# nianticlabs/simplerecon

Hardware: AMD Instinct MI355X
Metric: depth frames/sec (640x480, 7 src views, 64 planes) (higher is better)
Workload: dtype f32

## Files before the change

### include/simplerecon_hip.h

```cpp
#ifndef SIMPLERECON_HIP_H_
#define SIMPLERECON_HIP_H_

#include <stddef.h>
#include <stdint.h>

#ifdef __cplusplus
extern "C" {
#endif

#define SR_OK 0
#define SR_ERR_INVALID_ARGUMENT 1
#define SR_ERR_UNSUPPORTED 2
#define SR_ERR_WORKSPACE_TOO_SMALL 3
#define SR_ERR_HIP_BASE 1000

enum {
  SR_OPT_MLP_SPLIT = 0, SR_OPT_WINO_SPLIT, SR_OPT_WINO_XCD, SR_OPT_WINO_STAGGER, SR_OPT_WINO_WG_PER_CU, SR_OPT_WINO_NT,
  SR_OPT_WINO_KSPLIT, SR_OPT_CONV_WINO, SR_OPT_CONV_TILE, SR_OPT_CONV_KSPLIT, SR_OPT_MLP_VEC_STORE, SR_OPT_MLP_XCD,
  SR_OPT_MLP_BWD_VALU, SR_OPT_T16_XCD, SR_OPT_POOL_BW, SR_OPT_POOL_XCD, SR_OPT_PW_NT, SR_OPT_PW_KS, SR_OPT_PT_CFG, SR_OPT_PT_KS,
  SR_OPT_DOT_LDS, SR_OPT_DOT_QUAD, SR_OPT_DOT_LDS_G, SR_OPT_DOT_LDS_CULL, SR_OPT_DOT_LDS_CAP, SR_OPT_UPSAMPLE_QUAD,
  SR_OPT_POOL_STREAM,
  SR_OPT_COUNT
};
int sr_option_count(void);
const char* sr_option_name(int id);
int sr_option_id(const char* name);
int sr_option_get(int id, int* value);
int sr_option_set(int id, int value, int* previous );
int sr_option_default(int id, int* value);

int sr_abi_version(void);

const char* sr_target_arch(void);


size_t sr_volume_workspace_bytes(int B, int K, int C, int h, int w);

int sr_volume_prepare(const float* src, const float* K_src, const float* T_src_cur,
                      const float* T_cur_src, int B, int K, int C, int h, int w, void* workspace,
                      size_t workspace_bytes, void* stream);

int sr_dot_volume_sweep(const float* cur, const float* invK_cur, const float* planes, int64_t ps_b,
                        int64_t ps_d, int64_t ps_y, int64_t ps_x, int B, int K, int C, int h, int w,
                        int D, float* out_cv, int64_t cv_sb, int64_t cv_sd, int64_t cv_sp,
                        float* out_lowest, uint8_t* out_mask, void* workspace,
                        size_t workspace_bytes, void* stream);

int sr_conv3x3_wino_io_nhwc_fwd(const void* in, int64_t in_batch_stride, int in_pix_stride, const float* packed_u,
                                const float* bias, const void* residual, int64_t res_batch_stride, int res_pix_stride,
                                void* out, int64_t out_batch_stride, int out_pix_stride, int B, int H, int W, int Cin,
                                int Cout, float leaky_slope, int io_dtype, void* stream);
int sr_pw_conv_io_nhwc_fwd(const void* in, int64_t in_batch_stride, int in_pix_stride, const float* packed_w,
                           const float* bias, const void* residual, int64_t res_batch_stride, int res_pix_stride, void* out,
                           int64_t out_batch_stride, int out_pix_stride, int B, int HW, int Cin, int Cout, float act_code,
                           int io_dtype, void* stream);

size_t sr_pw_conv_tiled_workspace_bytes(int M, int Cin, int Cout);
int sr_pw_conv_tiled_plan(int M, int Cin, int Cout, int can_split, int* cfg, int* ks);
int sr_pw_conv_tiled_nhwc_fwd(const float* in, int in_pix_stride, const float* packed_w, const float* bias,
                              const float* gate, const float* residual, int res_pix_stride, float* out,
                              int out_pix_stride, int M, int HW, int Cin, int Cout, float act_code, void* workspace,
                              size_t workspace_bytes, void* stream);
int sr_pw_conv_supported(int Cin, int Cout);
int sr_pw_conv_plan(int B, int HW, int Cin, int Cout, int* nt, int* ks);
int sr_pw_conv_nhwc_fwd(const float* in, int64_t in_batch_stride, int in_pix_stride, const float* packed_w,
                        const float* bias, const float* gate, const float* residual, int64_t res_batch_stride,
                        int res_pix_stride, float* out, int64_t out_batch_stride, int out_pix_stride, int B, int HW,
                        int Cin, int Cout, float act_code, void* stream);

int sr_backproject_fwd(const float* depth, const float* invK, float* out_points, int B, int h, int w, void* stream);
int sr_project3d_fwd(const float* points, const float* K, const float* T, float* out, int B, int N, float eps,
                     void* stream);
int sr_backproject_bwd(const float* grad_points, const float* invK, float* grad_depth, int B, int h, int w, void* stream);
int sr_project3d_bwd(const float* grad_out, const float* points, const float* K, const float* T, float* grad_points, int B,
                     int N, float eps, void* stream);
int sr_pose_distance_fwd(const float* T, float* out, int n, void* stream);
int sr_camera_rays_fwd(const float* points, const float* T, float* out, int B, int N, int in_camera_frame, void* stream);

int sr_selftest_rcp(const float* x, float* out_fast, float* out_div, int n, void* stream);

int sr_dot_volume_fwd(const float* cur, const float* src, const float* K_src,
                      const float* T_src_cur, const float* invK_cur, const float* planes,
                      int64_t ps_b, int64_t ps_d, int64_t ps_y, int64_t ps_x, int B, int K, int C,
                      int h, int w, int D, float* out_cv, int64_t cv_sb, int64_t cv_sd,
                      int64_t cv_sp, float* out_lowest, uint8_t* out_mask, void* workspace,
                      size_t workspace_bytes, void* stream);

int sr_warp_features_fwd(const float* src, const float* K_src, const float* T_src_cur,
                         const float* invK_cur, const float* planes, int64_t ps_b, int64_t ps_d,
                         int64_t ps_y, int64_t ps_x, int B, int K, int C, int h, int w, int Dp,
                         float* out_world, float* out_depths, float* out_warped, float* out_mask,
                         float* out_pix, void* workspace, size_t workspace_bytes, void* stream);

size_t sr_mlp_volume_workspace_bytes(int B, int K, int C, int h, int w, int hidden);

int sr_mlp_pack_weights(const float* W1, const float* b1, const float* W2, const float* b2,
                        const float* W3, const float* b3, int hidden, int B, int K, int C, int h, int w,
                        void* workspace, size_t workspace_bytes, void* stream);

int sr_mlp_volume_sweep(const float* cur, const float* invK_cur, const float* planes, int64_t ps_b,
                        int64_t ps_d, int64_t ps_y, int64_t ps_x, float leaky_slope, int B, int K,
                        int C, int h, int w, int D, float* out_cv, int64_t cv_sb, int64_t cv_sd,
                        int64_t cv_sp, float* out_lowest, uint8_t* out_mask, void* workspace,
                        size_t workspace_bytes, void* stream);

int sr_mlp_volume_fwd(const float* cur, const float* src, const float* K_src, const float* T_src_cur,
                      const float* T_cur_src, const float* invK_cur, const float* planes, int64_t ps_b,
                      int64_t ps_d, int64_t ps_y, int64_t ps_x, const float* W1, const float* b1,
                      const float* W2, const float* b2, const float* W3, const float* b3, int hidden,
                      float leaky_slope, int B, int K, int C, int h, int w, int D, float* out_cv,
                      int64_t cv_sb, int64_t cv_sd, int64_t cv_sp, float* out_lowest, uint8_t* out_mask,
                      int reserve_cus, void* workspace, size_t workspace_bytes, void* stream);


size_t sr_conv_packed_weight_floats(int Cout, int Cin, int ksize);
// ... 232 lines not shown
```

### simplerecon_amd/_lib.py

```python
import contextlib
import ctypes as C
import os

import torch

_HERE = os.path.dirname(os.path.abspath(__file__))
LIB_PATH = os.environ.get("SR_HIP_LIBRARY") or os.path.join(_HERE, "libsimplerecon_hip.so")
ABI_VERSION = 3

_lib = None

_p = C.c_void_p
_i = C.c_int
_i64 = C.c_int64
_f = C.c_float
_sz = C.c_size_t

SIGNATURES = {
    "sr_abi_version": (_i, []),
    "sr_option_count": (_i, []),
    "sr_option_name": (C.c_char_p, [_i]),
    "sr_option_id": (_i, [C.c_char_p]),
    "sr_option_get": (_i, [_i, C.POINTER(C.c_int)]),
    "sr_option_set": (_i, [_i, _i, C.POINTER(C.c_int)]),
    "sr_option_default": (_i, [_i, C.POINTER(C.c_int)]),
    "sr_target_arch": (C.c_char_p, []),
    "sr_volume_workspace_bytes": (_sz, [_i, _i, _i, _i, _i]),
    "sr_volume_prepare": (_i, [_p, _p, _p, _p, _i, _i, _i, _i, _i, _p, _sz, _p]),
    "sr_dot_volume_sweep": (_i, [_p, _p, _p, _i64, _i64, _i64, _i64, _i, _i, _i, _i, _i, _i,
                                 _p, _i64, _i64, _i64, _p, _p, _p, _sz, _p]),
    "sr_dot_volume_fwd": (_i, [_p, _p, _p, _p, _p, _p, _i64, _i64, _i64, _i64, _i, _i, _i, _i, _i, _i,
                               _p, _i64, _i64, _i64, _p, _p, _p, _sz, _p]),
    "sr_rgb_stem3x3s2_fwd": (_i, [_p, _i64, _i64, _i64, _i64, _p, _p, _p, _i64, _i, _i, _i, _i, _i, _i, _i, _i, _i, _f, _p]),
    "sr_se_gate2_fwd": (_i, [_p, _i, _i, _p, _p, _p, _p, _p, _p, _i, _i, _i, _p]),
    "sr_conv3x3_wino_io_nhwc_fwd": (_i, [_p, _i64, _i, _p, _p, _p, _i64, _i, _p, _i64, _i, _i, _i, _i, _i, _i, _f, _i, _p]),
    "sr_pw_conv_io_nhwc_fwd": (_i, [_p, _i64, _i, _p, _p, _p, _i64, _i, _p, _i64, _i, _i, _i, _i, _i, _f, _i, _p]),
    "sr_pw_conv_tiled_workspace_bytes": (_sz, [_i, _i, _i]),
    "sr_pw_conv_tiled_plan": (_i, [_i, _i, _i, _i, _p, _p]),
    "sr_pw_conv_tiled_nhwc_fwd": (_i, [_p, _i, _p, _p, _p, _p, _i, _p, _i, _i, _i, _i, _i, _f, _p, _sz, _p]),
    "sr_pw_conv_supported": (_i, [_i, _i]),
    "sr_pw_conv_plan": (_i, [_i, _i, _i, _i, _p, _p]),
    "sr_pw_conv_nhwc_fwd": (_i, [_p, _i64, _i, _p, _p, _p, _p, _i64, _i, _p, _i64, _i, _i, _i, _i, _i, _f, _p]),
    "sr_backproject_fwd": (_i, [_p, _p, _p, _i, _i, _i, _p]),
    "sr_project3d_fwd": (_i, [_p, _p, _p, _p, _i, _i, _f, _p]),
    "sr_backproject_bwd": (_i, [_p, _p, _p, _i, _i, _i, _p]),
    "sr_project3d_bwd": (_i, [_p, _p, _p, _p, _p, _i, _i, _f, _p]),
    "sr_pose_distance_fwd": (_i, [_p, _p, _i, _p]),
    "sr_camera_rays_fwd": (_i, [_p, _p, _p, _i, _i, _i, _p]),
    "sr_selftest_rcp": (_i, [_p, _p, _p, _i, _p]),
    "sr_warp_features_fwd": (_i, [_p, _p, _p, _p, _p, _i64, _i64, _i64, _i64, _i, _i, _i, _i, _i, _i,
                                  _p, _p, _p, _p, _p, _p, _sz, _p]),
    "sr_mlp_volume_workspace_bytes": (_sz, [_i, _i, _i, _i, _i, _i]),
    "sr_mlp_pack_weights": (_i, [_p, _p, _p, _p, _p, _p, _i, _i, _i, _i, _i, _i, _p, _sz, _p]),
    "sr_mlp_volume_sweep": (_i, [_p, _p, _p, _i64, _i64, _i64, _i64, _f, _i, _i, _i, _i, _i, _i,
                                 _p, _i64, _i64, _i64, _p, _p, _p, _sz, _p]),
    "sr_mlp_volume_fwd": (_i, [_p, _p, _p, _p, _p, _p, _p, _i64, _i64, _i64, _i64, _p, _p, _p, _p, _p, _p, _i,
                               _f, _i, _i, _i, _i, _i, _i, _p, _i64, _i64, _i64, _p, _p, _i, _p, _sz, _p]),
    "sr_conv_packed_weight_floats": (_sz, [_i, _i, _i]),
    "sr_conv_pack_weights": (_i, [_p, _i, _i, _i, _p, _p]),
    "sr_conv2d_nhwc_fwd": (_i, [_p, _i64, _i, _p, _p, _p, _i64, _i, _p, _i64, _i, _i, _i, _i, _i, _i, _i, _i, _f, _p]),
    "sr_conv2d_replicate_nhwc_fwd": (_i, [_p, _i64, _i, _p, _p, _p, _i64, _i, _p, _i64, _i, _i, _i, _i, _i, _i, _i, _i,
                                          _f, _p]),
    "sr_conv2d_padded_nhwc_fwd": (_i, [_p, _i64, _i, _p, _p, _p, _i64, _i, _p, _i64, _i, _i, _i, _i, _i, _i, _i, _i,
                                       _i, _i, _i, _i, _f, _p]),
    "sr_dwconv3x3_pool_bands": (_i, [_i]),
    "sr_dwconv3x3_nhwc_fwd": (_i, [_p, _i64, _i, _p, _p, _p, _i64, _i, _p, _i, _i, _i, _i, _i, _i, _i, _i, _i, _f,
                                   _p]),
    "sr_add_nhwc_fwd": (_i, [_p, _i64, _i, _p, _i64, _i, _p, _i64, _i, _i, _i, _i, _i, _p]),
    "sr_se_scale_nhwc_fwd": (_i, [_p, _i, _p, _p, _p, _p, _p, _p, _i64, _i, _p, _i64, _i, _p, _i, _i, _i, _i, _i,
                                  _p]),
    "sr_se_gate_fwd": (_i, [_p, _i, _i, _p, _p, _p, _p, _p, _i, _i, _i, _p]),
    "sr_scale_channels_nhwc_fwd": (_i, [_p, _i64, _i, _p, _p, _i64, _i, _i, _i, _i, _i, _p]),
    "sr_dot_volume_bwd_scratch_bytes": (_sz, [_i, _i, _i, _i, _i]),
    "sr_dot_volume_bwd": (_i, [_p, _i64, _i64, _i64, _p, _p, _p, _i64, _i64, _i64, _i64, _i, _i, _i, _i, _i, _i, _p, _p,
                               _p, _sz, _p, _sz, _p]),
    "sr_mlp_volume_bwd_scratch_bytes": (_sz, [_i, _i, _i, _i, _i, _i]),
    "sr_mlp_volume_bwd": (_i, [_p, _i64, _i64, _i64, _p, _p, _p, _i64, _i64, _i64, _i64, _p, _p, _p, _p, _p, _f, _i, _i,
                               _i, _i, _i, _i, _i, _p, _p, _p, _p, _p, _p, _p, _p, _p, _sz, _p, _sz, _p]),
    "sr_conv_wgrad_workspace_bytes": (_sz, [_i, _i, _i, _i, _i, _i, _i]),
    "sr_conv_wgrad_nhwc": (_i, [_p, _i64, _i, _p, _i64, _i, _p, _i, _i, _i, _i, _i, _i, _i, _p, _sz, _p]),
    "sr_bias_grad_nhwc": (_i, [_p, _i64, _i, _p, _i, _i, _i, _i, _p]),
    "sr_act_bwd": (_i, [_p, _p, _p, _i64, _f, _p]),
    "sr_act_bwd_bias_workspace_bytes": (_sz, [_i64, _i]),
    "sr_act_bwd_bias_nhwc": (_i, [_p, _p, _p, _p, _i64, _i, _f, _p, _sz, _p]),
    "sr_zero_stuff2x_nhwc": (_i, [_p, _i64, _i, _p, _i, _i, _i, _i, _i, _i, _p]),
    "sr_upsample2x_bwd_nhwc": (_i, [_p, _i64, _i, _p, _i64, _i, _i, _i, _i, _i, _p]),
    "sr_conv_flip_transpose_weights": (_i, [_p, _i, _i, _i, _p, _p]),
    "sr_mul_fwd": (_i, [_p, _p, _p, _i64, _p]),
    "sr_norm_workspace_bytes": (_sz, [_i, _i, _i, _i]),
    "sr_norm_stats_nhwc": (_i, [_p, _i64, _i, _i, _i, _i, _i, _p, _p, _p, _sz, _p]),
    "sr_norm_act_fwd_nhwc": (_i, [_p, _i64, _i, _p, _p, _f, _p, _p, _f, _i, _p, _i64, _i, _i, _i, _i, _p]),
    "sr_norm_act_bwd_nhwc": (_i, [_p, _i64, _i, _p, _i64, _i, _p, _p, _f, _p, _p, _f, _i, _i, _p, _i64, _i, _p, _p,
# ... 208 lines not shown
```

### simplerecon_amd/csrc/sr_options.hip

```cpp
#include <atomic>
#include <mutex>
#include <stdlib.h>
#include <string.h>

#include "sr_common.h"

namespace {

struct OptDef { const char* name; int dflt; int kind; };
const OptDef kDefs[SR_OPT_COUNT] = {
    {"SR_MLP_SPLIT", 0, 1},       {"SR_WINO_SPLIT", 0, 1},     {"SR_WINO_XCD", 1, 0},        {"SR_WINO_STAGGER", 0, 0},
    {"SR_WINO_WG_PER_CU", 2, 0},  {"SR_WINO_NT", 0, 0},        {"SR_WINO_KSPLIT", 0, 0},     {"SR_CONV_WINO", 1, 0},
    {"SR_CONV_TILE", 0, 0},       {"SR_CONV_KSPLIT", 1, 0},    {"SR_MLP_VEC_STORE", 1, 0},   {"SR_MLP_XCD", 1, 0},
    {"SR_MLP_BWD_VALU", 0, 0},    {"SR_T16_XCD", 1, 0},        {"SR_POOL_BW", 0, 0},         {"SR_POOL_XCD", 1, 0},
    {"SR_PW_NT", 0, 0},           {"SR_PW_KS", 0, 0},          {"SR_PT_CFG", -1, 0},         {"SR_PT_KS", 0, 0},
    {"SR_DOT_LDS", 1, 0},         {"SR_DOT_QUAD", 1, 0},       {"SR_DOT_LDS_G", 0, 0},       {"SR_DOT_LDS_CULL", 1, 0},
    {"SR_DOT_LDS_CAP", 634, 0},   {"SR_UPSAMPLE_QUAD", 1, 0},  {"SR_POOL_STREAM", 1, 0},
};
std::atomic<int> g_val[SR_OPT_COUNT];
std::once_flag g_once;

int parse(const OptDef& d, const char* e) {
  if (d.kind == 1) {
    if (!e || !*e || !strcmp(e, "0") || !strcmp(e, "off") || !strcmp(e, "fp32")) return 0;
    if (!strcmp(e, "bf16")) return 1;
    if (!strcmp(e, "f16") || !strcmp(e, "fp16")) return 2;
    return -1;
  }
  return (e && *e) ? atoi(e) : d.dflt;
}

void init() {
  for (int i = 0; i < SR_OPT_COUNT; ++i) {
    const char* e = getenv(kDefs[i].name);
    g_val[i].store(e ? parse(kDefs[i], e) : kDefs[i].dflt, std::memory_order_relaxed);
  }
}

}

int sr_opt(int id) {
  std::call_once(g_once, init);
  return g_val[id].load(std::memory_order_relaxed);
}

extern "C" int sr_option_count(void) { return SR_OPT_COUNT; }

extern "C" const char* sr_option_name(int id) { return (id >= 0 && id < SR_OPT_COUNT) ? kDefs[id].name : nullptr; }

extern "C" int sr_option_id(const char* name) {
  if (!name) return -1;
  for (int i = 0; i < SR_OPT_COUNT; ++i)
    if (!strcmp(kDefs[i].name, name)) return i;
  return -1;
}

extern "C" int sr_option_get(int id, int* value) {
  if (id < 0 || id >= SR_OPT_COUNT || !value) return SR_ERR_INVALID_ARGUMENT;
  *value = sr_opt(id);
  return SR_OK;
}

extern "C" int sr_option_set(int id, int value, int* previous) {
  if (id < 0 || id >= SR_OPT_COUNT) return SR_ERR_INVALID_ARGUMENT;
  std::call_once(g_once, init);
  const int old = g_val[id].exchange(value, std::memory_order_relaxed);
  if (previous) *previous = old;
  return SR_OK;
}

// ... 19 lines not shown
```

### simplerecon_amd/ops.py

```python
import ctypes as C
import contextlib
import os
import weakref

import torch
from torch import nn

from . import _lib

PROFILE = None

_PACKED = weakref.WeakKeyDictionary()
_NO_ENTRIES = {}


def _cached(mod, tag, key, build, *args):
    e = _PACKED.get(mod, _NO_ENTRIES).get(tag)
    if e is not None and e[0] == key:
        if e[2] is not None:
            _await_pack(e)
        return e[1]
    payload = build(*args)
    fence = None
    if _lib.cuda_available() and not _lib.capturing():
# ... 94 lines not shown
        return (w._version, w.data_ptr(), b._version, b.data_ptr())
    ts = [w] if b is None else [w, b]
    bufs, bp = bn._buffers, bn._parameters
    ts += [bufs["running_mean"], bufs["running_var"]]
    if bn.affine:
        ts += [bp["weight"], bp["bias"]]
    return tuple((t._version, t.data_ptr()) if t is not None else None for t in ts)


def bn_affine(bn):
    if bn.running_mean is None or bn.running_var is None:
        raise _lib.HipLibraryError("BatchNorm without running statistics cannot run in inference mode")
    scale = torch.rsqrt(bn.running_var.detach() + bn.eps)
    if bn.affine:
        scale = scale * bn.weight.detach()
    shift = -bn.running_mean.detach() * scale
    if bn.affine:
        shift = shift + bn.bias.detach()
    return scale.contiguous(), shift.contiguous()


def _effective_weight(conv, bn):
    w = conv.weight.detach()
    b = conv.bias.detach() if conv.bias is not None else None
    if bn is not None:
        scale, shift = bn_affine(bn)
        w = w * scale.view(-1, 1, 1, 1)
        b = shift if b is None else b * scale + shift
    return w.contiguous(), b


def _check_conv(conv):
    k = conv.kernel_size[0]
    if conv.kernel_size[0] != conv.kernel_size[1] or k not in (1, 3) or conv.groups != 1 \
            or conv.dilation != (1, 1) or tuple(conv.padding) != (k // 2,) * 2 \
            or conv.padding_mode not in ("zeros", "replicate"):
        raise _lib.HipLibraryError(f"unsupported Conv2d configuration for the HIP path: {conv}")


def _pack_folded(kind, conv, bn):
    _lib.require_device_f32("conv weight", conv.weight)
    _check_conv(conv)
    w, bias = _effective_weight(conv, bn)
    return _pack(kind, w), bias


def packed_weight(conv: nn.Conv2d, bn=None):
    return _cached(conv, "direct", _state_key(conv, bn), _pack_folded, "conv", conv, bn)


USE_PW_1X1 = True
PW_TILED = os.environ.get("SR_PW_TILED", "auto")
PW_TILED_MIN_ROWS = 100000


def _pack_linear(lin):
    return _pack("conv", lin.weight.detach().reshape(lin.out_features, lin.in_features, 1, 1).contiguous())


def linear(x, lin: nn.Linear, leaky=None):
    _lib.require_device_f32("linear input", x)
    _lib.refuse_autograd(x, lin.weight)
    cin, cout = lin.in_features, lin.out_features
    if x.shape[-1] != cin:
        raise ValueError(f"linear expects {cin} input features, got {x.shape[-1]}")
    x2 = x.reshape(-1, cin).contiguous()
    m = x2.shape[0]
    out = torch.empty((m, cout), dtype=torch.float32, device=x.device)
    if m == 0:
        return out.view(*x.shape[:-1], cout)
    wp = _cached(lin, "linear", _state_key(lin, None), _pack_linear, lin)
    bias = lin.bias.detach() if lin.bias is not None else None
    lib = _lib.lib()
    with _lib.on_device(x.device):
        rc = lib.sr_conv2d_nhwc_fwd(_lib.ptr(x2), m * cin, cin, _lib.ptr(wp), _lib.ptr(bias), None, 0, 0,
                                    _lib.ptr(out), m * cout, cout, 1, 1, m, cin, cout, 1, 1,
                                    C.c_float(-1.0 if leaky is None else float(leaky)), _lib.stream_ptr(x.device))
    _lib.check(rc, "sr_conv2d_nhwc_fwd (linear)")
    return out.view(*x.shape[:-1], cout)


def wino_split_mode():
    return _lib.split_mode_name("SR_WINO_SPLIT")


def packed_wino_weight(conv: nn.Conv2d, bn=None):
    key = (_state_key(conv, bn), wino_split_mode())
    return _cached(conv, "wino", key, _pack_folded, "wino", conv, bn)


WINO4_MODE = int(os.environ.get("SR_CONV_WINO4", "1"))
WINO4_VARIANT = int(os.environ.get("SR_WINO4_VARIANT", "0"))


def packed_wino4_weight(conv: nn.Conv2d, bn=None):
    return _cached(conv, "wino4", _state_key(conv, bn), _pack_folded, "wino4", conv, bn)


_SHAPE_QUERIES = {}


def _drop_shape_queries(*_):
    _SHAPE_QUERIES.clear()


_lib.OPTION_LISTENERS.append(_drop_shape_queries)
# ... 96 lines not shown
    with _lib.on_device(device):
        if prof is None:
            return fn(*args)
        ev0, ev1 = torch.cuda.Event(enable_timing=True), torch.cuda.Event(enable_timing=True)
        ev0.record()
        rc = fn(*args)
        ev1.record()
        if rc == 0:
            name, flops, shape, executed = record()
            prof.append((name, flops, ev0, ev1, shape, executed))
    return rc


def _launch(x, shape, entry, fallback, describe, fn, *args):
    if PROFILE is None:
        with _lib.on_device(x.device):
            rc = fn(*args)
    else:
        def record():
            b, ci, h, w, co, k, s, ho, wo, _ = shape
            name, executed = describe()
            return name, 2.0 * b * ho * wo * co * ci * k * k, shape, executed
        rc = _timed(x.device, record, fn, *args)
    if rc != 0 and (rc != _lib.ERR_UNSUPPORTED or not fallback):
        _lib.check(rc, entry)
    return rc


def _conv_pointwise(lib, x, conv, bn, residual, out, gate, strides, shape, slope):
    isb, isp, osb, osp, rsb, rsp = strides
    b, ci, h, w, co = shape[:5]
    wp, bias = packed_weight(conv, bn)
    m = b * h * w
    dense = b == 1 or (isb == h * w * isp and osb == h * w * osp and (residual is None or rsb == h * w * rsp))
    gflag = "true" if gate is not None else "false"
    if dense and (PW_TILED == "1" or (PW_TILED == "auto" and m >= PW_TILED_MIN_ROWS)):
        nbytes = _shape_query(lib, "sr_pw_conv_tiled_workspace_bytes", m, ci, co, dev=x.device.index)
        ws = _workspace(x.device, "pw_splitk", nbytes) if nbytes else None

        def describe():
            a_, b_ = C.c_int(0), C.c_int(0)
            can_split = ws is not None and ws.data_ptr() % 16 == 0 and co % 4 == 0 and _aligned16(out, 0, osp) and \
                _aligned16(residual, 0, rsp) and (bias is None or bias.data_ptr() % 16 == 0)
            lib.sr_pw_conv_tiled_plan(m, ci, co, int(can_split), C.byref(a_), C.byref(b_))
            if b_.value > 1 and nbytes < b_.value * m * co * 4:
                lib.sr_pw_conv_tiled_plan(m, ci, co, 0, C.byref(a_), C.byref(b_))
            tile_m, tile_n = ((64, 128), (128, 160), (128, 64), (64, 64))[a_.value]
            executed = 2.0 * (-(-m // tile_m) * tile_m) * (-(-co // tile_n) * tile_n) * (-(-ci // 32) * 32)
            return f"sr_pw_tiled_kernel<{tile_m}x{tile_n}, ks {b_.value}, {gflag}>", executed
        return _launch(x, shape, "sr_pw_conv_tiled_nhwc_fwd", gate is None, describe, lib.sr_pw_conv_tiled_nhwc_fwd,
                       _lib.ptr(x), isp, _lib.ptr(wp), _lib.ptr(bias), _lib.ptr(gate), _lib.ptr(residual), rsp, _lib.ptr(out),
                       osp, m, h * w, ci, co, slope, _lib.ptr(ws), nbytes, _lib.stream_ptr(x.device))

    def describe():
        a_, b_ = C.c_int(0), C.c_int(0)
        lib.sr_pw_conv_plan(b, h * w, ci, co, C.byref(a_), C.byref(b_))
        mt = b * ((h * w + 31) // 32)
        executed = 2.0 * mt * 32 * ((co + 32 * a_.value - 1) // (32 * a_.value) * 32 * a_.value) * ((ci + 7) // 8 * 8)
        return f"sr_pw_kernel<{a_.value}, {b_.value}, {gflag}>", executed
    return _launch(x, shape, "sr_pw_conv_nhwc_fwd", gate is None, describe, lib.sr_pw_conv_nhwc_fwd, _lib.ptr(x), isb, isp,
                   _lib.ptr(wp), _lib.ptr(bias), _lib.ptr(gate), _lib.ptr(residual), rsb, rsp, _lib.ptr(out), osb, osp, b,
                   h * w, ci, co, slope, _lib.stream_ptr(x.device))


def _conv_wino4(lib, x, conv, bn, residual, out, strides, shape, slope, variant):
    isb, isp, osb, osp, rsb, rsp = strides
    b, ci, h, w, co = shape[:5]
    wp, bias = packed_wino4_weight(conv, bn)
    if not (_aligned16(x, isb, isp) and _aligned16(out, osb, osp) and _aligned16(residual, rsb, rsp)
            and (bias is None or bias.data_ptr() % 16 == 0)):
        return _lib.ERR_UNSUPPORTED

    def describe():
        regions = ((h + 15) // 16) * ((w + 15) // 16)
        executed = 2.0 * b * regions * 16 * 36 * ((ci + 15) // 16 * 16) * ((co + 63) // 64 * 64)
        return "sr_wino4ws_kernel" if variant == 3 else "sr_wino4_kernel", executed
    return _launch(x, shape, "sr_conv3x3_wino4_nhwc_fwd", True, describe, lib.sr_conv3x3_wino4_variant_nhwc_fwd, _lib.ptr(x),
                   isb, isp, _lib.ptr(wp), _lib.ptr(bias), _lib.ptr(residual), rsb, rsp, _lib.ptr(out), osb, osp, b, h, w, ci,
                   co, slope, variant, _lib.stream_ptr(x.device))


def _conv_wino(lib, x, conv, bn, residual, out, strides, shape, slope):
    isb, isp, osb, osp, rsb, rsp = strides
    b, ci, h, w, co = shape[:5]
    split = wino_split_mode()
    wp, bias = packed_wino_weight(conv, bn)
    nbytes = _shape_query(lib, "sr_wino_splitk_workspace_bytes", b, h, w, ci, co, dev=x.device.index)
    ws = _workspace(x.device, "wino_splitk", nbytes) if nbytes else None

    def describe():
        vin = bool(_aligned16(x, isb, isp) and ci % 4 == 0)
        vout = vin and co % 4 == 0 and _aligned16(out, osb, osp) and _aligned16(residual, rsb, rsp) and \
            (bias is None or bias.data_ptr() % 16 == 0)
        name = lib.sr_wino_kernel_name(b, h, w, ci, co, int(vin), int(vout)).decode()
        if split:
            name = name.replace("sr_wino_kernel<", "sr_wino_split_kernel<").replace(
                ", true, true>", f", {1 if split == 'bf16' else 2}>")
        regions = ((h + 7) // 8) * ((w + 15) // 16)
        return name, 2.0 * b * regions * 32 * 16 * ((ci + 15) // 16 * 16) * ((co + 31) // 32 * 32)
    return _launch(x, shape, "sr_conv3x3_wino_nhwc_fwd", not split, describe, lib.sr_conv3x3_wino_splitk_nhwc_fwd,
                   _lib.ptr(x), isb, isp, _lib.ptr(wp), _lib.ptr(bias), _lib.ptr(residual), rsb, rsp, _lib.ptr(out), osb, osp,
                   b, h, w, ci, co, slope, _lib.ptr(ws), nbytes, _lib.stream_ptr(x.device))


def _conv_direct(lib, x, conv, bn, residual, out, strides, shape, slope, pads, replicate):
    isb, isp, osb, osp, rsb, rsp = strides
# ... 13 lines not shown
    return launch(lib.sr_conv2d_splitk_nhwc_fwd, slope, _lib.ptr(ws), nbytes)


def basic_block(block, x, out=None):
    if not isinstance(block.bn1, nn.Identity) or not isinstance(block.bn2, nn.Identity):
        raise _lib.HipLibraryError("the HIP BasicBlock implements norm_layer=nn.Identity only (what SimpleRecon uses)")
    slope = block.relu.negative_slope
    x = as_nhwc(x, "BasicBlock input")
    t = conv2d(x, block.conv1, leaky=slope)
    identity = x if block.downsample is None else conv2d(x, block.downsample[0])
    return conv2d(t, block.conv2, residual=identity, leaky=slope, out=out)


def upsample2x(x, out=None):
    x = as_nhwc(x, "upsample input")
    _lib.refuse_autograd(x)
    b, c, h, w = x.shape
    if out is None:
        out = empty_nhwc(b, c, 2 * h, 2 * w, x.device)
    elif tuple(out.shape) != (b, c, 2 * h, 2 * w) or not _is_nhwc_view(out):
        raise ValueError(f"`out` must be a channels-last view of shape {(b, c, 2 * h, 2 * w)}")
    if b == 0:
        return out
    isb, isp = _strides(x)
    osb, osp = _strides(out)
    with _lib.on_device(x.device):
        rc = _lib.lib().sr_upsample2x_nhwc_fwd(_lib.ptr(x), isb, isp, _lib.ptr(out), osb, osp, b, h, w, c,
                                               _lib.stream_ptr(x.device))
    _lib.check(rc, "sr_upsample2x_nhwc_fwd")
    return out


def exp(x):
    _lib.require_device_f32("exp input", x)
    if not (x.is_contiguous() or x.is_contiguous(memory_format=torch.channels_last)):
        x = x.contiguous()
    out = torch.empty_like(x)
    with _lib.on_device(x.device):
        rc = _lib.lib().sr_exp_fwd(_lib.ptr(x), _lib.ptr(out), x.numel(), _lib.stream_ptr(x.device))
    _lib.check(rc, "sr_exp_fwd")
    return out


def copy_into(dst_view, src):
    _lib.require_device_f32("copy source", src)
    dst_view.copy_(src)
    return dst_view



_WORKSPACES = {}


def _workspace(device, tag, nbytes):
    if _lib.capturing():
        return torch.empty((nbytes + 3) // 4, dtype=torch.float32, device=device)
    key = (device, tag, _lib.stream_id(device))
    ws = _WORKSPACES.get(key)
    if ws is None or ws.numel() * 4 < nbytes:
        ws = torch.empty((nbytes + 3) // 4, dtype=torch.float32, device=device)
        _WORKSPACES[key] = ws
    return ws


def _pack_stem(conv, bn):
    wp = _pack("stem", conv.weight.detach().contiguous())
    scale = shift = None
    if bn is not None:
        scale, shift = bn_affine(bn)
    if conv.bias is not None:
        cb = conv.bias.detach()
        shift = (cb if scale is None else cb * scale) + (0 if shift is None else shift)
        shift = shift.contiguous()
    return wp, scale, shift


def stem7x7(image, conv: nn.Conv2d, bn=None, leaky=0.0, out=None):
    _lib.require_device_f32("image", image)
    _lib.refuse_autograd(image, conv.weight)
    if conv.kernel_size != (7, 7) or conv.stride != (2, 2) or tuple(conv.padding) != (3, 3) or conv.groups != 1 \
            or conv.dilation != (1, 1) or conv.in_channels != 3 or conv.out_channels != 64 \
            or conv.padding_mode != "zeros":
        raise _lib.HipLibraryError(f"the HIP stem implements Conv2d(3, 64, 7, stride=2, padding=3) only, got {conv}")
    if image.dim() != 4 or image.shape[1] != 3:
        raise ValueError(f"stem expects [B,3,H,W], got {tuple(image.shape)}")
    _lib.require_device_f32("stem weight", conv.weight)
    wp, scale, shift = _cached(conv, "stem", _state_key(conv, bn), _pack_stem, conv, bn)
    b, _, h, w = image.shape
    ho, wo = (h - 1) // 2 + 1, (w - 1) // 2 + 1
    if out is None:
        out = empty_nhwc(b, 64, ho, wo, image.device)
    elif tuple(out.shape) != (b, 64, ho, wo) or not _is_nhwc_view(out):
        raise ValueError(f"`out` must be a channels-last view of shape {(b, 64, ho, wo)}")
    if b == 0:
        return out
    sb, sc, sy, sx = image.stride()
    osb, osp = _strides(out)
    record = lambda: ("sr_stem_kernel", 2.0 * b * ho * wo * 64 * 147, (b, 3, h, w, 64, 7, 2),
                      2.0 * b * ((ho + 15) // 16) * ((wo + 15) // 16) * 256 * 64 * 148)
    rc = _timed(image.device, record, _lib.lib().sr_stem7x7_fwd, _lib.ptr(image), sb, sc, sy, sx, _lib.ptr(wp),
                _lib.ptr(scale), _lib.ptr(shift), C.c_float(-1.0 if leaky is None else float(leaky)), _lib.ptr(out), osb,
                osp, b, h, w, 64, _lib.stream_ptr(image.device))
    _lib.check(rc, "sr_stem7x7_fwd")
    return out


def maxblurpool(x, out=None):
    x = as_nhwc(x, "maxblurpool input")
    b, c, h, w = x.shape
    if h < 4 or w < 4:
        raise ValueError(f"maxblurpool needs H, W >= 4, got {(h, w)}")
    ho, wo = (h - 2) // 2 + 1, (w - 2) // 2 + 1
    if out is None:
# ... 296 lines not shown
```

Before: 313.6.

## Add MFMA split-K pointwise conv kernel for wide-input 1x1 convolutions

Adds a new 1x1 convolution kernel that uses fp32 MFMA 16x16x4 instructions with buffer loads and double-buffered operand fetch. For large Cin it splits K across waves, reduced in LDS, and across workgroups, where the last arriving workgroup reduces partials through a ticket counter. It is routed in only for Cin>=1024 and Cout>=128 in auto mode, aimed at the few wide pointwise layers (likely the cost-volume MLP or encoder heads) that the older kernel handled poorly. It adds a zeroed counter workspace and partial buffers, plus the risk of ordering bugs in the last-block reduction.

```diff
diff --git a/include/simplerecon_hip.h b/include/simplerecon_hip.h
--- a/include/simplerecon_hip.h
+++ b/include/simplerecon_hip.h
@@ -19,7 +19,7 @@
   SR_OPT_WINO_KSPLIT, SR_OPT_CONV_WINO, SR_OPT_CONV_TILE, SR_OPT_CONV_KSPLIT, SR_OPT_MLP_VEC_STORE, SR_OPT_MLP_XCD,
   SR_OPT_MLP_BWD_VALU, SR_OPT_T16_XCD, SR_OPT_POOL_BW, SR_OPT_POOL_XCD, SR_OPT_PW_NT, SR_OPT_PW_KS, SR_OPT_PT_CFG, SR_OPT_PT_KS,
   SR_OPT_DOT_LDS, SR_OPT_DOT_QUAD, SR_OPT_DOT_LDS_G, SR_OPT_DOT_LDS_CULL, SR_OPT_DOT_LDS_CAP, SR_OPT_UPSAMPLE_QUAD,
-  SR_OPT_POOL_STREAM,
+  SR_OPT_POOL_STREAM, SR_OPT_PW_RB, SR_OPT_PW_RB_NB, SR_OPT_PW_RB_KC, SR_OPT_PW_RB_KW,
   SR_OPT_COUNT
 };
 int sr_option_count(void);
@@ -61,6 +61,14 @@
                               const float* gate, const float* residual, int res_pix_stride, float* out,
                               int out_pix_stride, int M, int HW, int Cin, int Cout, float act_code, void* workspace,
                               size_t workspace_bytes, void* stream);
+int sr_pw_rb_plan(int Cin, int Cout, int* nb, int* kw, int* chunk_channels);
+size_t sr_pw_rb_workspace_bytes(int B, int HW, int Cin, int Cout);
+size_t sr_pw_rb_counter_bytes(int B, int HW, int Cin, int Cout);
+int sr_pw_rb_nhwc_fwd(const float* in, int64_t in_batch_stride, int in_pix_stride, const float* packed_w,
+                      const float* bias, const float* gate, const float* residual, int64_t res_batch_stride,
+                      int res_pix_stride, float* out, int64_t out_batch_stride, int out_pix_stride, int B, int HW,
+                      int Cin, int Cout, float act_code, void* workspace, size_t workspace_bytes, void* counters,
+                      size_t counter_bytes, void* stream);
 int sr_pw_conv_supported(int Cin, int Cout);
 int sr_pw_conv_plan(int B, int HW, int Cin, int Cout, int* nt, int* ks);
 int sr_pw_conv_nhwc_fwd(const float* in, int64_t in_batch_stride, int in_pix_stride, const float* packed_w,
diff --git a/simplerecon_amd/_lib.py b/simplerecon_amd/_lib.py
--- a/simplerecon_amd/_lib.py
+++ b/simplerecon_amd/_lib.py
@@ -38,6 +38,11 @@
     "sr_pw_conv_tiled_workspace_bytes": (_sz, [_i, _i, _i]),
     "sr_pw_conv_tiled_plan": (_i, [_i, _i, _i, _i, _p, _p]),
     "sr_pw_conv_tiled_nhwc_fwd": (_i, [_p, _i, _p, _p, _p, _p, _i, _p, _i, _i, _i, _i, _i, _f, _p, _sz, _p]),
+    "sr_pw_rb_plan": (_i, [_i, _i, _p, _p, _p]),
+    "sr_pw_rb_workspace_bytes": (_sz, [_i, _i, _i, _i]),
+    "sr_pw_rb_counter_bytes": (_sz, [_i, _i, _i, _i]),
+    "sr_pw_rb_nhwc_fwd": (_i, [_p, _i64, _i, _p, _p, _p, _p, _i64, _i, _p, _i64, _i, _i, _i, _i, _i, _f, _p, _sz, _p, _sz,
+                               _p]),
     "sr_pw_conv_supported": (_i, [_i, _i]),
     "sr_pw_conv_plan": (_i, [_i, _i, _i, _i, _p, _p]),
     "sr_pw_conv_nhwc_fwd": (_i, [_p, _i64, _i, _p, _p, _p, _p, _i64, _i, _p, _i64, _i, _i, _i, _i, _i, _f, _p]),
diff --git a/simplerecon_amd/csrc/sr_options.hip b/simplerecon_amd/csrc/sr_options.hip
--- a/simplerecon_amd/csrc/sr_options.hip
+++ b/simplerecon_amd/csrc/sr_options.hip
@@ -16,6 +16,8 @@
     {"SR_PW_NT", 0, 0},           {"SR_PW_KS", 0, 0},          {"SR_PT_CFG", -1, 0},         {"SR_PT_KS", 0, 0},
     {"SR_DOT_LDS", 1, 0},         {"SR_DOT_QUAD", 1, 0},       {"SR_DOT_LDS_G", 0, 0},       {"SR_DOT_LDS_CULL", 1, 0},
     {"SR_DOT_LDS_CAP", 634, 0},   {"SR_UPSAMPLE_QUAD", 1, 0},  {"SR_POOL_STREAM", 1, 0},
+    {"SR_PW_RB", 1, 0},           {"SR_PW_RB_NB", 0, 0},       {"SR_PW_RB_KC", 0, 0},
+    {"SR_PW_RB_KW", 0, 0},
 };
 std::atomic<int> g_val[SR_OPT_COUNT];
 std::once_flag g_once;
diff --git a/simplerecon_amd/csrc/sr_pw_rb.hip b/simplerecon_amd/csrc/sr_pw_rb.hip
--- /dev/null
+++ b/simplerecon_amd/csrc/sr_pw_rb.hip
@@ -0,0 +1,308 @@
+#include <stdint.h>
+
+#include "sr_common.h"
+
+namespace {
+
+typedef float rb_f4 __attribute__((ext_vector_type(4)));
+typedef unsigned int rb_u4 __attribute__((ext_vector_type(4)));
+typedef __attribute__((address_space(1))) unsigned rb_gu32;
+#define RB_RSRC_FLAGS 0x00020000
+#define RB_OOB 0x7fffffffu
+#define RB_SC1 16
+
+__device__ __forceinline__ __amdgpu_buffer_rsrc_t rb_rsrc(const void* base, int64_t bytes) {
+  return __builtin_amdgcn_make_buffer_rsrc(const_cast<void*>(base), 0, (int)bytes, RB_RSRC_FLAGS);
+}
+template <int AUX = 0>
+__device__ __forceinline__ rb_f4 rb_load(__amdgpu_buffer_rsrc_t r, unsigned voff, unsigned soff) {
+  return __builtin_bit_cast(rb_f4, __builtin_amdgcn_raw_buffer_load_b128(r, (int)voff, (int)soff, AUX));
+}
+
+struct SrPwRbParams {
+  const float* in; int64_t in_sb; int in_sp;
+  const float* wp;
+  const float* bias;
+  const float* gate;
+  const float* res; int64_t res_sb; int res_sp;
+  float* out; int64_t out_sb; int out_sp;
+  float* part;
+  unsigned* cnt;
+  int HW, Cin, Cout, Co_pad, G, G16;
+  int m_tiles, n_tiles, n_grps, chunks, cg;
+  float slope;
+};
+
+template <int NB, int KW, bool GATE>
+__global__ __launch_bounds__(256, 2) void sr_pw_rb_kernel(SrPwRbParams p) {
+  constexpr int NA = 4 * NB;
+  extern __shared__ __attribute__((aligned(16))) rb_f4 red[];
+  const int tid = threadIdx.x;
+  const int lane = tid & 63, wave = __builtin_amdgcn_readfirstlane(tid >> 6);
+  const int i = lane & 15, kq = lane >> 4;
+  const int item = blockIdx.x;
+  const int kp = wave % KW;
+  const int nt = (item % p.n_grps) * (4 / KW) + wave / KW;
+  const int c = (item / p.n_grps) % p.chunks;
+  const int mt_g = item / (p.n_grps * p.chunks);
+  if (KW == 1 && nt >= p.n_tiles) return;
+  const int tile = mt_g * p.n_tiles + nt;
+  const int img = mt_g / p.m_tiles;
+  const int row0 = (mt_g - img * p.m_tiles) * 64;
+  const int n0 = nt * 16 * NB;
+
+  const int cg0 = c * p.cg;
+  const int len = min(p.G16, cg0 + p.cg) - cg0;
+  const int per = len / KW, extra = len % KW;
+  const int g0 = cg0 + kp * per + min(kp, extra);
+  const int steps = per + (kp < extra ? 1 : 0);
+
+  const __amdgpu_buffer_rsrc_t rs_in = rb_rsrc(p.in + (int64_t)img * p.in_sb, ((int64_t)(p.HW - 1) * p.in_sp + p.Cin) * 4);
+  const __amdgpu_buffer_rsrc_t rs_w = rb_rsrc(p.wp, (int64_t)p.G * 2 * p.Co_pad * 16);
+  const __amdgpu_buffer_rsrc_t rs_g = rb_rsrc(GATE ? p.gate + (int64_t)img * p.Cin : p.wp, GATE ? (int64_t)p.Cin * 4 : 0);
+  unsigned a_voff[4];
+#pragma unroll
+  for (int mb = 0; mb < 4; ++mb) {
+    const int row = row0 + 16 * mb + i;
+    a_voff[mb] = row < p.HW ? ((unsigned)row * (unsigned)p.in_sp + 4u * kq) * 4u : RB_OOB;
+  }
+  unsigned w_voff[NB];
+#pragma unroll
+  for (int nb = 0; nb < NB; ++nb) {
+    const int col = n0 + 16 * nb + i;
+    w_voff[nb] = col < p.Co_pad ? ((unsigned)kq * (unsigned)p.Co_pad + (unsigned)col) * 16u : RB_OOB;
+  }
+  const unsigned w_gstride = 4u * (unsigned)p.Co_pad * 16u;
+  const bool k_tail = (p.Cin & 15) != 0;
+
+  rb_f4 acc[4][NB];
+#pragma unroll
+  for (int mb = 0; mb < 4; ++mb)
+#pragma unroll
+    for (int nb = 0; nb < NB; ++nb) acc[mb][nb] = rb_f4{0.0f, 0.0f, 0.0f, 0.0f};
+
+  rb_f4 a_f[2][4], b_f[2][NB], s_f[2];
+  auto issue = [&](int g, int slot) {
+    const bool kin = !k_tail || 16 * g + 4 * kq + 4 <= p.Cin;
+#pragma unroll
+    for (int mb = 0; mb < 4; ++mb) a_f[slot][mb] = rb_load(rs_in, kin ? a_voff[mb] : RB_OOB, (unsigned)g * 64u);
+    if (GATE) s_f[slot] = rb_load(rs_g, 16u * kq + (unsigned)g * 64u, 0u);
+#pragma unroll
+    for (int nb = 0; nb < NB; ++nb) b_f[slot][nb] = rb_load(rs_w, w_voff[nb], (unsigned)g * w_gstride);
+    __builtin_amdgcn_sched_barrier(0);
+  };
+  auto mma = [&](int slot) {
+    rb_f4 a[4];
+#pragma unroll
+    for (int mb = 0; mb < 4; ++mb) a[mb] = GATE ? a_f[slot][mb] * s_f[slot] : a_f[slot][mb];
+#pragma unroll
+    for (int e = 0; e < 4; ++e)
+#pragma unroll
+      for (int mb = 0; mb < 4; ++mb)
+#pragma unroll
+        for (int nb = 0; nb < NB; ++nb)
+          acc[mb][nb] = __builtin_amdgcn_mfma_f32_16x16x4f32(a[mb][e], b_f[slot][nb][e], acc[mb][nb], 0, 0, 0);
+  };
+  if (steps > 0) issue(g0, 0);
+  int s = 0;
+  for (; s + 2 <= steps; s += 2) {
+    issue(g0 + s + 1, 1);
+    mma(0);
+    issue(g0 + min(s + 2, steps - 1), 0);
+    mma(1);
+  }
+  if (s < steps) mma(0);
+
+  if (KW > 1) {
+    if (wave > 0) {
+#pragma unroll
+      for (int mb = 0; mb < 4; ++mb)
+#pragma unroll
+        for (int nb = 0; nb < NB; ++nb) red[((wave - 1) * NA + mb * NB + nb) * 64 + lane] = acc[mb][nb];
+    }
+    __syncthreads();
+    if (wave > 0) return;
+#pragma unroll
+    for (int q = 0; q < KW - 1; ++q)
+#pragma unroll
+      for (int mb = 0; mb < 4; ++mb)
+#pragma unroll
+        for (int nb = 0; nb < NB; ++nb) acc[mb][nb] += red[(q * NA + mb * NB + nb) * 64 + lane];
+  }
+
+  if (p.chunks > 1) {
+    const int64_t slab = (int64_t)NA * 64;
+    const __amdgpu_buffer_rsrc_t rs_p =
+        rb_rsrc(reinterpret_cast<rb_f4*>(p.part) + (int64_t)tile * p.chunks * slab, (int64_t)p.chunks * slab * 16);
+#pragma unroll
+    for (int a = 0; a < NA; ++a)
+      __builtin_amdgcn_raw_buffer_store_b128(__builtin_bit_cast(rb_u4, acc[a / NB][a % NB]), rs_p,
+                                             (int)(((unsigned)c * NA + a) * 64u + lane) * 16, 0, RB_SC1);
+    asm volatile("s_waitcnt vmcnt(0)" ::: "memory");
+    unsigned ticket = 0;
+    if (lane == 0) ticket = __hip_atomic_fetch_add((rb_gu32*)(p.cnt + tile), 1u, __ATOMIC_RELAXED, __HIP_MEMORY_SCOPE_AGENT);
+    ticket = __builtin_amdgcn_readfirstlane(ticket);
+    if (ticket != (unsigned)(p.chunks - 1)) return;
+    if (lane == 0) __hip_atomic_store((rb_gu32*)(p.cnt + tile), 0u, __ATOMIC_RELAXED, __HIP_MEMORY_SCOPE_AGENT);
+    __builtin_amdgcn_fence(__ATOMIC_ACQUIRE, "wavefront");
+    for (int q = 0; q < p.chunks; ++q) {
+      rb_f4 v[NA];
+#pragma unroll
+      for (int a = 0; a < NA; ++a) v[a] = rb_load<RB_SC1>(rs_p, (((unsigned)q * NA + a) * 64u + lane) * 16u, 0u);
+      if (q == 0) {
+#pragma unroll
+        for (int a = 0; a < NA; ++a) acc[a / NB][a % NB] = v[a];
+      } else {
+#pragma unroll
+        for (int a = 0; a < NA; ++a) acc[a / NB][a % NB] += v[a];
+      }
+    }
+  }
+
+  const float slope = sr_uniform(p.slope);
+  const __amdgpu_buffer_rsrc_t rs_out =
+      rb_rsrc(p.out + (int64_t)img * p.out_sb, ((int64_t)(p.HW - 1) * p.out_sp + p.Cout) * 4);
+  const bool has_res = p.res != nullptr;
+  const __amdgpu_buffer_rsrc_t rs_res =
+      rb_rsrc(has_res ? (const void*)(p.res + (int64_t)img * p.res_sb) : (const void*)p.wp,
+              has_res ? ((int64_t)(p.HW - 1) * p.res_sp + p.Cout) * 4 : (int64_t)0);
+#pragma unroll
+  for (int nb = 0; nb < NB; ++nb) {
+    const int col = n0 + 16 * nb + i;
+    const bool okc = col < p.Cout;
+    const float bv = (p.bias && okc) ? p.bias[col] : 0.0f;
+    float v[16];
+#pragma unroll
+    for (int mb = 0; mb < 4; ++mb)
+#pragma unroll
+      for (int r = 0; r < 4; ++r) v[mb * 4 + r] = acc[mb][nb][r] + bv;
+    if (has_res) {
+      float rv[16];
+#pragma unroll
+      for (int q = 0; q < 16; ++q) {
+        const int row = row0 + 16 * (q >> 2) + 4 * kq + (q & 3);
+        const bool ok = okc && row < p.HW;
+        rv[q] = __builtin_bit_cast(float, __builtin_amdgcn_raw_buffer_load_b32(
+            rs_res, ok ? (int)(((unsigned)row * (unsigned)p.res_sp + (unsigned)col) * 4u) : (int)RB_OOB, 0, 0));
+      }
+#pragma unroll
+      for (int q = 0; q < 16; ++q) v[q] += rv[q];
+    }
+    sr_activate_group(v, slope);
+#pragma unroll
+    for (int q = 0; q < 16; ++q) {
+      const int row = row0 + 16 * (q >> 2) + 4 * kq + (q & 3);
+      const bool ok = okc && row < p.HW;
+      __builtin_amdgcn_raw_buffer_store_b32(__builtin_bit_cast(unsigned, v[q]), rs_out,
+                                            ok ? (int)(((unsigned)row * (unsigned)p.out_sp + (unsigned)col) * 4u) : (int)RB_OOB,
+                                            0, 0);
+    }
+  }
+}
+
+struct RbPlan { int nb, kw, cg; };
+
+RbPlan rb_plan(int Cin, int Cout) {
+  const int f_nb = sr_opt(SR_OPT_PW_RB_NB), f_kc = sr_opt(SR_OPT_PW_RB_KC), f_kw = sr_opt(SR_OPT_PW_RB_KW);
+  if (Cin <= 0 || Cout <= 0 || Cin % 4 != 0 || sr_opt(SR_OPT_PW_RB) <= 0) return {0, 0, 0};
+  const int g16 = (Cin + 15) / 16;
+  const int nb = (f_nb == 4 || f_nb == 5) ? f_nb : ((Cout + 79) / 80 * 80 <= (Cout + 63) / 64 * 64 ? 5 : 4);
+  const int kw = (f_kw == 1 || f_kw == 4) ? f_kw : (g16 <= 20 ? 1 : 4);
+  int cg;
+  if (f_kc > 0) {
+    cg = min((f_kc + 15) / 16, g16);
+  } else if (kw == 1) {
+    cg = g16;
+  } else {
+    const int chunks = (g16 + 31) / 32;
+    cg = (g16 + chunks - 1) / chunks;
+  }
+  return {nb, kw, cg};
+}
+
+struct RbShape { int m_tiles, n_tiles, n_grps, chunks; int64_t tiles; };
+RbShape rb_shape(const RbPlan& pl, int B, int HW, int Cin, int Cout) {
+  RbShape s;
+  s.m_tiles = (HW + 63) / 64;
+  s.n_tiles = (Cout + 16 * pl.nb - 1) / (16 * pl.nb);
+  s.n_grps = (s.n_tiles + 4 / pl.kw - 1) / (4 / pl.kw);
+  s.chunks = ((Cin + 15) / 16 + pl.cg - 1) / pl.cg;
+  s.tiles = (int64_t)B * s.m_tiles * s.n_tiles;
+  return s;
+}
+
+template <int NB, int KW>
+int rb_launch(const SrPwRbParams& p, int64_t wgs, hipStream_t stream) {
+  const size_t lds = (size_t)(KW - 1) * 4 * NB * 64 * 16;
+  if (p.gate) hipLaunchKernelGGL((sr_pw_rb_kernel<NB, KW, true>), dim3((unsigned)wgs), dim3(256), lds, stream, p);
+  else hipLaunchKernelGGL((sr_pw_rb_kernel<NB, KW, false>), dim3((unsigned)wgs), dim3(256), lds, stream, p);
+  return sr_hip_rc(hipGetLastError());
+}
+
+}
+
+extern "C" int sr_pw_rb_plan(int Cin, int Cout, int* nb, int* kw, int* chunk_channels) {
+  const RbPlan pl = rb_plan(Cin, Cout);
+  if (nb) *nb = pl.nb;
+  if (kw) *kw = pl.kw;
+  if (chunk_channels) *chunk_channels = 16 * pl.cg;
+  return pl.cg > 0 ? 1 : 0;
+}
+
+extern "C" size_t sr_pw_rb_workspace_bytes(int B, int HW, int Cin, int Cout) {
+  const RbPlan pl = rb_plan(Cin, Cout);
+  if (pl.cg <= 0 || B <= 0 || HW <= 0) return 0;
+  const RbShape s = rb_shape(pl, B, HW, Cin, Cout);
+  return s.chunks > 1 ? (size_t)s.tiles * s.chunks * 4 * pl.nb * 64 * 16 : 0;
+}
+
+extern "C" size_t sr_pw_rb_counter_bytes(int B, int HW, int Cin, int Cout) {
+  const RbPlan pl = rb_plan(Cin, Cout);
+  if (pl.cg <= 0 || B <= 0 || HW <= 0) return 0;
+  const RbShape s = rb_shape(pl, B, HW, Cin, Cout);
+  return s.chunks > 1 ? sr_align_up((size_t)s.tiles * 4, 256) : 0;
+}
+
+extern "C" int sr_pw_rb_nhwc_fwd(const float* in, int64_t in_batch_stride, int in_pix_stride, const float* packed_w,
+                                 const float* bias, const float* gate, const float* residual, int64_t res_batch_stride,
+                                 int res_pix_stride, float* out, int64_t out_batch_stride, int out_pix_stride, int B, int HW,
+                                 int Cin, int Cout, float act_code, void* workspace, size_t workspace_bytes,
+                                 void* counters, size_t counter_bytes, void* stream_) {
+  if (B < 0 || HW <= 0 || Cin <= 0 || Cout <= 0) return SR_ERR_INVALID_ARGUMENT;
+  if (B == 0) return SR_OK;
+  if (!in || !packed_w || !out) return SR_ERR_INVALID_ARGUMENT;
+  const RbPlan pl = rb_plan(Cin, Cout);
+  if (pl.cg <= 0) return SR_ERR_UNSUPPORTED;
+  if (in_pix_stride % 4 != 0 || in_batch_stride % 4 != 0 || (((uintptr_t)in) & 15) != 0 ||
+      (gate && (((uintptr_t)gate) & 15) != 0))
+    return SR_ERR_UNSUPPORTED;
+  const int64_t lim = (int64_t)1 << 31;
+  if (((int64_t)(HW - 1) * in_pix_stride + Cin) * 4 >= lim || ((int64_t)(HW - 1) * out_pix_stride + Cout) * 4 >= lim ||
+      (residual && ((int64_t)(HW - 1) * res_pix_stride + Cout) * 4 >= lim))
+    return SR_ERR_UNSUPPORTED;
+  const RbShape s = rb_shape(pl, B, HW, Cin, Cout);
+  if (s.chunks > 1) {
+    if (!workspace || !counters || (((uintptr_t)workspace) & 15) != 0 || (((uintptr_t)counters) & 3) != 0 ||
+        workspace_bytes < sr_pw_rb_workspace_bytes(B, HW, Cin, Cout) ||
+        counter_bytes < (size_t)s.tiles * 4)
+      return SR_ERR_INVALID_ARGUMENT;
+    if ((int64_t)s.chunks * 4 * pl.nb * 64 * 16 >= lim) return SR_ERR_UNSUPPORTED;
+  }
+  const int64_t wgs = (int64_t)B * s.m_tiles * s.n_grps * s.chunks;
+  if (wgs >= lim) return SR_ERR_UNSUPPORTED;
+  SrPwRbParams p;
+  p.in = in; p.in_sb = in_batch_stride; p.in_sp = in_pix_stride;
+  p.wp = packed_w; p.bias = bias; p.gate = gate;
+  p.res = residual; p.res_sb = res_batch_stride; p.res_sp = res_pix_stride;
+  p.out = out; p.out_sb = out_batch_stride; p.out_sp = out_pix_stride;
+  p.part = (float*)workspace; p.cnt = (unsigned*)counters;
+  p.HW = HW; p.Cin = Cin; p.Cout = Cout;
+  p.Co_pad = ((Cout + 31) / 32) * 32;
+  p.G = ((Cin + 63) / 64) * 8;
+  p.G16 = (Cin + 15) / 16;
+  p.m_tiles = s.m_tiles; p.n_tiles = s.n_tiles; p.n_grps = s.n_grps; p.chunks = s.chunks; p.cg = pl.cg;
+  p.slope = act_code;
+  hipStream_t stream = (hipStream_t)stream_;
+  if (pl.kw == 1) return pl.nb == 5 ? rb_launch<5, 1>(p, wgs, stream) : rb_launch<4, 1>(p, wgs, stream);
+  return pl.nb == 5 ? rb_launch<5, 4>(p, wgs, stream) : rb_launch<4, 4>(p, wgs, stream);
+}
diff --git a/simplerecon_amd/ops.py b/simplerecon_amd/ops.py
--- a/simplerecon_amd/ops.py
+++ b/simplerecon_amd/ops.py
@@ -170,6 +170,8 @@
 USE_PW_1X1 = True
 PW_TILED = os.environ.get("SR_PW_TILED", "auto")
 PW_TILED_MIN_ROWS = 100000
+PW_RB_MIN_CIN = 1024
+PW_RB_MIN_CHANNELS = 128
 
 
 def _pack_linear(lin):
@@ -372,6 +374,22 @@
                        _lib.ptr(x), isp, _lib.ptr(wp), _lib.ptr(bias), _lib.ptr(gate), _lib.ptr(residual), rsp, _lib.ptr(out),
                        osp, m, h * w, ci, co, slope, _lib.ptr(ws), nbytes, _lib.stream_ptr(x.device))
 
+    if PW_TILED == "auto" and ci >= PW_RB_MIN_CIN and co >= PW_RB_MIN_CHANNELS and _shape_query(lib, "sr_pw_rb_plan", ci, co, None, None, None):
+        nbytes = _shape_query(lib, "sr_pw_rb_workspace_bytes", b, h * w, ci, co)
+        cbytes = _shape_query(lib, "sr_pw_rb_counter_bytes", b, h * w, ci, co)
+        ws = _workspace(x.device, "pw_rb", nbytes) if nbytes else None
+        cnt = _workspace(x.device, "pw_rb_cnt", cbytes, zero=True) if cbytes else None
+
+        def describe():
+            nb_, kw_, kc_ = C.c_int(0), C.c_int(0), C.c_int(0)
+            lib.sr_pw_rb_plan(ci, co, C.byref(nb_), C.byref(kw_), C.byref(kc_))
+            tn = 16 * nb_.value
+            executed = 2.0 * b * (-(-(h * w) // 64) * 64) * (-(-co // tn) * tn) * (-(-ci // 16) * 16)
+            return f"sr_pw_rb_kernel<{nb_.value}, kw {kw_.value}, kc {kc_.value}, {gflag}>", executed
+        return _launch(x, shape, "sr_pw_rb_nhwc_fwd", gate is None, describe, lib.sr_pw_rb_nhwc_fwd, _lib.ptr(x), isb, isp,
+                       _lib.ptr(wp), _lib.ptr(bias), _lib.ptr(gate), _lib.ptr(residual), rsb, rsp, _lib.ptr(out), osb, osp,
+                       b, h * w, ci, co, slope, _lib.ptr(ws), nbytes, _lib.ptr(cnt), cbytes, _lib.stream_ptr(x.device))
+
     def describe():
         a_, b_ = C.c_int(0), C.c_int(0)
         lib.sr_pw_conv_plan(b, h * w, ci, co, C.byref(a_), C.byref(b_))
@@ -491,13 +509,14 @@
 _WORKSPACES = {}
 
 
-def _workspace(device, tag, nbytes):
+def _workspace(device, tag, nbytes, zero=False):
+    alloc = torch.zeros if zero else torch.empty
     if _lib.capturing():
-        return torch.empty((nbytes + 3) // 4, dtype=torch.float32, device=device)
+        return alloc((nbytes + 3) // 4, dtype=torch.float32, device=device)
     key = (device, tag, _lib.stream_id(device))
     ws = _WORKSPACES.get(key)
     if ws is None or ws.numel() * 4 < nbytes:
-        ws = torch.empty((nbytes + 3) // 4, dtype=torch.float32, device=device)
+        ws = alloc((nbytes + 3) // 4, dtype=torch.float32, device=device)
         _WORKSPACES[key] = ws
     return ws
 
```

New measurement: 314.5 (median of 6 runs). No clear change (+0.3%).
